# wwood/CoverM

Hardware: NVIDIA H100
Metric: reads/sec `coverm contig` (mean+trimmed_mean+covered_fraction) (higher is better)
Workload: dtype i32

## Files before the change

### coverm_b200/csrc/cmb_bgzf.cu

```cuda
#include <algorithm>
#include <atomic>
#include <chrono>
#include <climits>
#include <cstdio>
#include <cstdlib>
#include <cstring>
#include <thread>

#include <zlib.h>

#include "cmb_context.cuh"
#include "cmb_bgzf.cuh"

namespace {
#include "cmb_common.cuh"
#include "cmb_decode.cuh"
#include "cmb_decode_g8.cuh"
#include "cmb_decode_t1.cuh"
#include "cmb_pairs.cuh"
#include "cmb_filter.cuh"
}

namespace {
constexpr size_t DEC_COPY_CHUNK = 8u << 20;
constexpr size_t DEC_WINDOW_BYTES = 32u << 20;
size_t dec_window_bytes() {
  static const size_t v = [] {
    const char* e = getenv("CMB_DECODE_WINDOW_KB");
    const long kb = e ? atol(e) : 0;
    return kb > 0 ? (size_t)kb << 10 : DEC_WINDOW_BYTES;
  }();
  return v;
}
constexpr size_t DEC_SLACK = 1024;
constexpr const char* NM_PANIC = "Mapping record encountered that does not have an 'NM' auxiliary tag in the SAM/BAM format. This is "
                                 "required to work out some coverage statistics";
constexpr size_t DEC_FRONT = 256;

constexpr uint32_t T1_MIN_BLOCKS = 28000;
int inflate_kind(uint32_t n_blocks) {
  static const int forced = [] {
    const char* e = getenv("CMB_INFLATE");
    if (e && !strcmp(e, "t1")) return 0;
    if (e && !strcmp(e, "g8")) return 1;
    if (e && !strcmp(e, "w1")) return 2;
    return -1;
  }();
  if (forced >= 0) return forced;
  return n_blocks >= T1_MIN_BLOCKS ? 0 : 1;
}
bool inflate_serial_requested() {
  static const bool v = [] {
    if (const char* e = getenv("CMB_INFLATE_SERIAL")) return e[0] == '1';
    for (const char* name : {"CUDA_INJECTION64_PATH", "NV_NSIGHT_INJECTION_PORT_BASE", "NV_COMPUTE_PROFILER_PERFWORKS_DIR", "NV_SANITIZER_INJECTION_PORT_BASE"})
      if (const char* e = getenv(name))
        if (e[0]) return true;
    return false;
  }();
  return v;
}
int launch_crc32(cmb_ctx* c, const InflateArgs& a, cudaStream_t st) {
  const uint32_t nb = a.b1 - a.b0;
  kd_crc32<<<std::min<uint32_t>((nb + 7) / 8, (uint32_t)c->sm_count * 8), 256, 0, st>>>(a);
  CU_TRY(c, cudaGetLastError());
  return CMB_OK;
}
int launch_inflate(cmb_ctx* c, const InflateArgs& a, cudaStream_t st, bool* crc_pending = nullptr) {
  const uint32_t nb = a.b1 - a.b0;
  const int k = a.block_list ? 2 : inflate_kind(nb);
  if (k == 0) {
    CU_TRY(c, cudaFuncSetAttribute(kd_inflate_t1, cudaFuncAttributeMaxDynamicSharedMemorySize, (int)T1_SMEM_BYTES));
    const uint32_t max_grid = (uint32_t)c->sm_count * 5, warps = max_grid * (T1_THREADS / 32);
    const uint32_t lanes = std::min<uint32_t>(32, std::max<uint32_t>(1, (nb + warps - 1) / warps));
    const uint32_t per_cta = lanes * (T1_THREADS / 32);
    const uint32_t grid = std::min<uint32_t>((nb + per_cta - 1) / per_cta, max_grid);
    InflateArgs at = a;
    at.lane_limit = lanes;
    kd_inflate_t1<<<grid, T1_THREADS, T1_SMEM_BYTES, st>>>(at);
    CU_TRY(c, cudaGetLastError());
    if (crc_pending) *crc_pending = true;
    else if (int rc = launch_crc32(c, a, st)) return rc;
  } else if (k == 1) {
    CU_TRY(c, cudaFuncSetAttribute(kd_inflate_g8, cudaFuncAttributeMaxDynamicSharedMemorySize, (int)G8_SMEM_BYTES));
    const uint32_t per_cta = G8_WARPS * G8_STREAMS;
    const uint32_t grid = std::min<uint32_t>((nb + per_cta - 1) / per_cta, (uint32_t)c->sm_count * 2);
    kd_inflate_g8<<<grid, G8_WARPS * 32, G8_SMEM_BYTES, st>>>(a);
  } else {
    CU_TRY(c, cudaFuncSetAttribute(kd_inflate, cudaFuncAttributeMaxDynamicSharedMemorySize, (int)INF_SMEM_BYTES));
    const uint32_t grid = std::min<uint32_t>((nb + INF_WARPS - 1) / INF_WARPS, (uint32_t)c->sm_count * 2);
    kd_inflate<<<grid, INF_WARPS * 32, INF_SMEM_BYTES, st>>>(a);
  }
  CU_TRY(c, cudaGetLastError());
  return CMB_OK;
}

bool host_inflate_block(const cmb_bgzf_input* in, uint32_t b, std::vector<uint8_t>& buf) {
  const uint32_t isz = in->block_isize[b];
  if (buf.size() < (size_t)isz + 64) buf.resize((size_t)isz + 64);
  z_stream zs;
  memset(&zs, 0, sizeof zs);
  if (inflateInit2(&zs, -15) != Z_OK) return false;
  zs.next_in = const_cast<Bytef*>(in->data + in->block_coffset[b]);
  zs.avail_in = in->block_clen[b];
  zs.next_out = buf.data();
  zs.avail_out = isz;
  const bool ok = inflate(&zs, Z_FINISH) == Z_STREAM_END && zs.avail_out == 0;
  inflateEnd(&zs);
  uint32_t want_crc;
  memcpy(&want_crc, in->data + in->block_coffset[b] + in->block_clen[b], 4);
  return ok && (uint32_t)crc32(0, buf.data(), isz) == want_crc;
}

InflateArgs inflate_args(const BgzfCall& j, uint32_t b0, uint32_t b1) {
  const auto& d = j.d;
  InflateArgs a{};
  a.comp = j.comp_base; a.coff = d.d_coff; a.clen = d.d_clen; a.isize = d.d_isize; a.uoff = d.d_ustart; a.scratch = d.d_t1_scratch;
  a.b0 = b0; a.b1 = b1; a.out = j.infl_base; a.status = d.d_status; a.ticket = d.d_tickets; a.fail_count = d.d_cnt + 0;
  return a;
}

}

std::optional<uint64_t> cmb::decode_mem_limit() {
  const char* lim = getenv("CMB_DECODE_MEM_LIMIT_MB");
  if (!lim) return std::nullopt;
  return (uint64_t)(std::max(0.0, strtod(lim, nullptr)) * 1048576.0);
}

uint64_t cmb::decode_bytes(const cmb_ctx* c) {
  const auto& d = c->dec;
  return d.d_comp.bytes() + d.d_inflated.bytes() + d.d_tuple_slab.bytes() + d.d_rec_off.bytes() + c->sh.d_scan.bytes();
}

void cmb::release_decode(cmb_ctx* c) {
  cudaGetLastError();
  auto& d = c->dec;
  d.d_comp.release();
  d.d_inflated.release();
  d.d_tuple_slab.release();
  d.d_rec_off.release();
  c->sh.d_scan.release();
}

uint64_t cmb::device_room(uint64_t held) {
  if (const uint64_t lim = decode_mem_limit().value_or(0)) return lim;
  size_t free_b = 0, total_b = 0;
  cudaMemGetInfo(&free_b, &total_b);
  cudaGetLastError();
  return free_b + held;
}


int BgzfCall::run() {
  int rc = prepare();
  if (!rc && !nothing_to_decode && !(rc = copy_inflate()) && !(rc = declined()) && !(rc = chain())) rc = extract();
  return rc;
}

int BgzfCall::prepare() {
  ustart.assign((size_t)nb + 1, 0);
  for (uint32_t b = 0; b < nb; ++b) {
    if (in->block_coffset[b] + in->block_clen[b] + 8 > in->size) return fail(c, CMB_E_ARG, "cmb_submit_bgzf: block %u lies outside the data", b);
    ustart[b + 1] = ustart[b] + in->block_isize[b];
  }
  const uint64_t stream_total = ustart[nb];
  if (in->records_at > stream_total) return fail(c, CMB_E_ARG, "cmb_submit_bgzf: records_at beyond the end of the stream");
  if (in->records_at == stream_total) return CMB_OK;
  first_block = (uint32_t)(std::upper_bound(ustart.begin(), ustart.end(), in->records_at) - ustart.begin()) - 1;
  walk_end = data_end = nb;
  if (in->ranged) {
    if (in->walk_begin_block != first_block || in->walk_end_block > nb || in->walk_end_block < in->walk_begin_block)
      return fail(c, CMB_E_ARG, "cmb_submit_bgzf: inconsistent block range");
    walk_end = in->walk_end_block;
    if (walk_end == first_block) return CMB_OK;
    data_end = walk_end;
    uint64_t tail = 0;
    while (data_end < nb && tail < tail_bytes) tail += in->block_isize[data_end++];
  }
  nothing_to_decode = false;
  byte_lo = in->block_coffset[first_block];
  byte_hi = data_end == nb ? in->size : in->block_coffset[data_end - 1] + in->block_clen[data_end - 1] + 8;
  u_lo = ustart[first_block];
  total = ustart[data_end];
  if (const auto lim = decode_mem_limit())
    if (((byte_hi - byte_lo) + (total - u_lo)) >> 20 > *lim >> 20) return CMB_E_NOMEM;
  int rc;
  const size_t comp_need = (size_t)(byte_hi - byte_lo) + DEC_FRONT + DEC_SLACK, infl_need = (size_t)(total - u_lo) + DEC_SLACK;
  if ((rc = d.d_comp.ensure(c, comp_need, with_slack(comp_need))) || (rc = d.d_inflated.ensure(c, infl_need, with_slack(infl_need))))
    return rc;
  comp_base = reinterpret_cast<uint8_t*>(reinterpret_cast<uintptr_t>(d.d_comp.p) + DEC_FRONT - byte_lo);
  infl_base = reinterpret_cast<uint8_t*>(reinterpret_cast<uintptr_t>(d.d_inflated.p) - u_lo);
  const size_t blocks_need = (size_t)nb + 1, blocks_want = (size_t)nb + nb / 8 + 64;
  for (auto* b : {&d.d_coff, &d.d_ustart, &d.d_guess, &d.d_exit, &d.d_rec_base, &d.d_cig_base})
    if ((rc = b->ensure(c, blocks_need, blocks_want))) return rc;
  for (auto* b : {&d.d_clen, &d.d_isize, &d.d_status, &d.d_nrec, &d.d_ncig, &d.d_dirty})
    if ((rc = b->ensure(c, blocks_need, blocks_want))) return rc;
  if ((rc = d.d_t1_scratch.ensure(c, blocks_need * T1_LENS_BYTES, blocks_want * T1_LENS_BYTES))) return rc;
  if ((rc = d.d_cnt.ensure(c, 20))) return rc;
  if (!d.have_events) {
    for (auto& e : d.ev) CU_TRY(c, cudaEventCreate(&e));
    d.have_events = true;
  }
  {
    uint32_t b = first_block;
    uint64_t byte0 = byte_lo;
    while (b < data_end) {
      uint32_t e = b;
      uint64_t byte1 = byte0;
      while (e < data_end && (e == b || in->block_coffset[e] + in->block_clen[e] + 8 - byte0 <= dec_window_bytes())) {
        byte1 = in->block_coffset[e] + in->block_clen[e] + 8;
        ++e;
      }
      if (e == data_end) byte1 = byte_hi;
      windows.push_back({b, e, byte0, byte1});
      b = e;
      byte0 = byte1;
    }
  }
  const size_t n_windows = windows.size();
  if ((rc = d.d_tickets.ensure(c, n_windows + 8, n_windows * 3 + 64))) return rc;
  if ((rc = d.d_block_window.ensure(c, nb, with_slack(nb)))) return rc;
  if (!d.h_ones) {
    if ((rc = d.h_ones.ensure(c, 16))) return rc;
    for (int k = 0; k < 16; ++k) d.h_ones.p[k] = 1;
  }
  cudaPointerAttributes attr{};
  src_pinned = cudaPointerGetAttributes(&attr, in->data) == cudaSuccess && attr.type == cudaMemoryTypeHost;
  cudaGetLastError();
  const uint32_t T = std::min<uint32_t>(std::min<uint32_t>(in->copy_threads ? in->copy_threads : 4, 16), (uint32_t)n_windows);
  n_copy_threads = T;
  while (d.streams.size() < T) {
    cudaStream_t st;
    CU_TRY(c, cudaStreamCreateWithFlags(&st, cudaStreamNonBlocking));
    d.streams.push_back(st);
    cudaEvent_t e;
    CU_TRY(c, cudaEventCreateWithFlags(&e, cudaEventDisableTiming));
    d.done_events.push_back(e);
    for (int k = 0; k < 2; ++k) {
      CU_TRY(c, cudaEventCreateWithFlags(&e, cudaEventDisableTiming));
      d.slot_events.push_back(e);
      PinnedBuf<uint8_t> slot;
      if ((rc = slot.ensure(c, DEC_COPY_CHUNK))) return rc;
      d.pinned.push_back(std::move(slot));
    }
  }
  return CMB_OK;
}

int BgzfCall::copy_inflate() {
  NvtxRange nvtx("bgzf: H2D copy + inflate");
  const uint32_t T = n_copy_threads;
  std::vector<uint32_t> block_window(nb, 0);
  for (size_t w = 0; w < windows.size(); ++w)
    for (uint32_t b = windows[w].b0; b < windows[w].b1; ++b) block_window[b] = (uint32_t)w;
  CU_TRY(c, cudaEventRecord(d.ev[0], c->stream));
  CU_TRY(c, cudaMemcpyAsync(d.d_coff, in->block_coffset, 8ull * nb, cudaMemcpyHostToDevice, c->stream));
  CU_TRY(c, cudaMemcpyAsync(d.d_clen, in->block_clen, 4ull * nb, cudaMemcpyHostToDevice, c->stream));
  CU_TRY(c, cudaMemcpyAsync(d.d_isize, in->block_isize, 4ull * nb, cudaMemcpyHostToDevice, c->stream));
  CU_TRY(c, cudaMemcpyAsync(d.d_ustart, ustart.data(), 8ull * (nb + 1), cudaMemcpyHostToDevice, c->stream));
  CU_TRY(c, cudaMemsetAsync(d.d_cnt, 0, 64, c->stream));
  CU_TRY(c, cudaMemsetAsync(d.d_status, 0, 4ull * nb, c->stream));
  CU_TRY(c, cudaMemcpyAsync(d.d_block_window, block_window.data(), 4ull * nb, cudaMemcpyHostToDevice, c->stream));
  CU_TRY(c, cudaMemsetAsync(d.d_tickets, 0, 4 * (windows.size() + 1), c->stream));
  CU_TRY(c, cudaMemsetAsync(infl_base + total, 0, DEC_SLACK, c->stream));
  CU_TRY(c, cudaMemsetAsync(comp_base + byte_hi, 0, DEC_SLACK, c->stream));
  CU_TRY(c, cudaMemsetAsync(d.d_comp, 0, DEC_FRONT, c->stream));
  CU_TRY(c, cudaEventRecord(d.ev[1], c->stream));
  for (uint32_t t = 0; t < T; ++t) CU_TRY(c, cudaStreamWaitEvent(d.streams[t], d.ev[1], 0));
  const bool serial = windows.size() <= 1 || inflate_serial_requested();
  bool crc_pending = false;
  InflateArgs persistent = inflate_args(*this, first_block, data_end);
  int rc;
  if (!serial) {
    persistent.block_window = d.d_block_window;
    persistent.ready = d.d_tickets + 1;
    if ((rc = launch_inflate(c, persistent, c->stream, &crc_pending))) return rc;
  }
  std::atomic<size_t> next_window{0};
  std::atomic<int> first_err{0};
  auto worker = [&](uint32_t t) {
    cudaSetDevice(c->device);
    cudaStream_t st = d.streams[t];
    int slot = 0;
    bool used[2] = {false, false};
    auto check = [&](cudaError_t e) {
      if (e != cudaSuccess) {
        int z = 0;
        first_err.compare_exchange_strong(z, (int)e);
      }
      return e == cudaSuccess;
    };
    for (;;) {
      const size_t w = next_window.fetch_add(1);
      if (w >= windows.size() || first_err.load()) break;
      const Window& win = windows[w];
      if (src_pinned) {
        if (!check(cudaMemcpyAsync(comp_base + win.byte0, in->data + win.byte0, win.byte1 - win.byte0, cudaMemcpyHostToDevice, st))) break;
      } else {
        for (uint64_t o = win.byte0; o < win.byte1; o += DEC_COPY_CHUNK) {
          const size_t n = (size_t)std::min<uint64_t>(DEC_COPY_CHUNK, win.byte1 - o);
          const size_t si = (size_t)t * 2 + slot;
          if (used[slot] && !check(cudaEventSynchronize(d.slot_events[si]))) return;
          memcpy(d.pinned[si], in->data + o, n);
          if (!check(cudaMemcpyAsync(comp_base + o, d.pinned[si], n, cudaMemcpyHostToDevice, st))) return;
          if (!check(cudaEventRecord(d.slot_events[si], st))) return;
          used[slot] = true;
          slot ^= 1;
        }
      }
      if (!check(cudaMemcpyAsync(d.d_tickets + 1 + w, d.h_ones, 4, cudaMemcpyHostToDevice, st))) break;
    }
    check(cudaEventRecord(d.done_events[t], st));
  };
  const auto copy_t0 = std::chrono::steady_clock::now();
  {
    std::vector<std::thread> threads;
    for (uint32_t t = 1; t < T; ++t) threads.emplace_back(worker, t);
    worker(0);
    for (auto& th : threads) th.join();
  }
  const double copy_wall_ms = std::chrono::duration<double, std::milli>(std::chrono::steady_clock::now() - copy_t0).count();
  out->ms_copy_enqueue_wall = (float)copy_wall_ms;
  if (crc_pending && (rc = launch_crc32(c, persistent, c->stream))) return rc;
  if (serial && !first_err.load()) {
    for (uint32_t t = 0; t < T; ++t) CU_TRY(c, cudaStreamWaitEvent(c->stream, d.done_events[t], 0));
    if ((rc = launch_inflate(c, inflate_args(*this, first_block, data_end), c->stream))) return rc;
  }
  if (first_err.load()) {
    cudaMemsetAsync(d.d_tickets + 1, 1, 4 * windows.size(), d.streams[0]);
    cudaStreamSynchronize(d.streams[0]);
    cudaStreamSynchronize(c->stream);
  }
  out->n_launches = 1;
  out->h2d_bytes = (byte_hi - byte_lo) + 24ull * nb + 8;
  if (first_err.load()) return fail(c, CMB_E_CUDA, "cmb_submit_bgzf: copy/inflate stage failed: %s", cudaGetErrorString((cudaError_t)first_err.load()));
  for (uint32_t t = 0; t < T; ++t) CU_TRY(c, cudaStreamWaitEvent(c->stream, d.done_events[t], 0));
  if (getenv("CMB_PIPELINE_STATS")) {
    const auto h0 = std::chrono::steady_clock::now();
    for (uint32_t t = 0; t < T; ++t) cudaEventSynchronize(d.done_events[t]);
    const double wait_ms = std::chrono::duration<double, std::milli>(std::chrono::steady_clock::now() - h0).count();
    fprintf(stderr, "#decode_h2d\twindows=%zu\tbytes=%llu\tcopy_streams_done_after_ms=%.1f (host clock from the end of the enqueue; enqueue took %.1f ms)\n",
            windows.size(), (unsigned long long)(byte_hi - byte_lo), wait_ms, copy_wall_ms);
  }
  CU_TRY(c, cudaEventRecord(d.ev[2], c->stream));
  if (getenv("CMB_DECODE_PROFILE")) {
    CU_TRY(c, cudaStreamSynchronize(c->stream));
    cudaEvent_t p0, p1;
    cudaEventCreate(&p0);
    cudaEventCreate(&p1);
    CU_TRY(c, cudaMemsetAsync(d.d_tickets, 0, 4, c->stream));
    InflateArgs a = inflate_args(*this, first_block, data_end);
    a.fail_count = d.d_cnt + 8;
    cudaEventRecord(p0, c->stream);
    if ((rc = launch_inflate(c, a, c->stream))) return rc;
    cudaEventRecord(p1, c->stream);
    CU_TRY(c, cudaStreamSynchronize(c->stream));
    float ms = 0;
    cudaEventElapsedTime(&ms, p0, p1);
    fprintf(stderr, "#decode_profile\tinflate_only_ms=%.3f\tblocks=%u\tcompressed=%llu\tinflated=%llu\tinflated_GBps=%.2f\tcopy_threads=%u\tsrc_pinned=%d\tcopy_enqueue_wall_ms=%.2f\n", ms, data_end - first_block,
            (unsigned long long)(byte_hi - byte_lo), (unsigned long long)(total - u_lo), (total - u_lo) / ms * 1e-6, T, (int)src_pinned, copy_wall_ms);
    cudaEventDestroy(p0);
    cudaEventDestroy(p1);
  }
  return CMB_OK;
}

int BgzfCall::declined() {
  NvtxRange nvtx("bgzf: declined blocks (second pass, host zlib)");
  uint32_t h_cnt[16];
  CU_TRY(c, cudaMemcpyAsync(h_cnt, d.d_cnt, 64, cudaMemcpyDeviceToHost, c->stream));
  CU_TRY(c, cudaStreamSynchronize(c->stream));
  std::vector<uint8_t> tmp;
  if (h_cnt[0] || getenv("CMB_DECODE_RETRY_TEST")) {
    std::vector<uint32_t> status(nb);
    CU_TRY(c, cudaMemcpy(status.data(), d.d_status, 4ull * nb, cudaMemcpyDeviceToHost));
    if (getenv("CMB_DECODE_RETRY_TEST"))
      for (uint32_t b = first_block; b < data_end; b += 7) status[b] = 29;
    if (getenv("CMB_DECODE_VERIFY") || getenv("CMB_PIPELINE_STATS")) {
      uint32_t hist[32] = {0};
      for (uint32_t b = 0; b < nb; ++b) hist[std::min<uint32_t>(status[b], 31)]++;
      fprintf(stderr, "#decode_status");
      for (int k = 0; k < 32; ++k)
        if (hist[k]) fprintf(stderr, "\t%d:%u", k, hist[k]);
      fprintf(stderr, "\n");
    }
    std::vector<uint32_t> again;
    for (uint32_t b = first_block; b < data_end; ++b)
      if (status[b] != INF_OK) again.push_back(b);
    out->n_blocks_second_pass = (uint32_t)again.size();
    if (!again.empty()) {
      uint32_t* d_list = d.d_dirty;
      CU_TRY(c, cudaMemcpyAsync(d_list, again.data(), 4ull * again.size(), cudaMemcpyHostToDevice, c->stream));
      CU_TRY(c, cudaMemsetAsync(d.d_tickets, 0, 4, c->stream));
      CU_TRY(c, cudaMemsetAsync(d.d_cnt, 0, 4, c->stream));
      InflateArgs a = inflate_args(*this, 0, (uint32_t)again.size());
      a.block_list = d_list;
      if (int rc = launch_inflate(c, a, c->stream)) return rc;
      out->n_launches += 1;
      std::vector<uint32_t> st2(nb);
      CU_TRY(c, cudaMemcpyAsync(st2.data(), d.d_status, 4ull * nb, cudaMemcpyDeviceToHost, c->stream));
      CU_TRY(c, cudaStreamSynchronize(c->stream));
      for (uint32_t b : again) status[b] = st2[b];
    }
    for (uint32_t b = first_block; b < data_end; ++b) {
      if (status[b] == INF_OK) continue;
      if (!host_inflate_block(in, b, tmp)) return fail(c, CMB_E_DECLINED, "cmb_submit_bgzf: BGZF block %u does not inflate", b);
      CU_TRY(c, cudaMemcpy(infl_base + ustart[b], tmp.data(), in->block_isize[b], cudaMemcpyHostToDevice));
      out->n_blocks_host += 1;
    }
  }
  if (getenv("CMB_DECODE_VERIFY")) {
    std::vector<uint8_t> dev(total - u_lo);
    CU_TRY(c, cudaMemcpy(dev.data(), d.d_inflated, total - u_lo, cudaMemcpyDeviceToHost));
    uint32_t bad = 0;
// ... 285 lines not shown
      if ((rc = pair_cut(j, filter_out, carry, j.walk_end >= walk_end, who, host_route, &largest, &cut, next))) return rc;
      ss.ms_mates += std::chrono::duration<float, std::milli>(std::chrono::steady_clock::now() - t0).count();
    }
    if ((rc = work(j, r, cut))) return rc;
    carry = largest;
    ss.pair_cut_records += n - cut;
    side = (double)other() / (double)std::max<uint64_t>(1, (j.byte_hi - j.byte_lo) + (j.total - j.u_lo));
    return CMB_OK;
  };
  auto nomem = [&](const SliceBlocks&, uint32_t, uint32_t, uint64_t) {
    return fail(c, CMB_E_DECLINED, "%s: not enough device memory for device-side decode", who);
  };
  const int rc = decode_in_slices(c, in, out, ss, budget, step, nomem);
  release_decode(c);
  if (rc) return rc;
  if (getenv("CMB_PIPELINE_STATS"))
    fprintf(stderr, "#%s_slices\tslices=%u\tmax_slice_bytes=%llu\thalvings=%u\tpair_cut_records=%llu\n", stats, ss.n_slices,
            (unsigned long long)ss.max_slice, ss.halvings, (unsigned long long)ss.pair_cut_records);
  return CMB_OK;
}

int decode_sliced(cmb_ctx* c, const cmb_bgzf_input* in, cmb_bgzf_result* out) {
  auto& d = c->dec;
  *out = cmb_bgzf_result{};
  const bool pair = c->mode.filter_pairs;
  auto work = [&](BgzfCall& j, cmb_bgzf_result& r, uint32_t cut) -> int {
    const uint32_t n = (uint32_t)j.n_rec;
    uint32_t iv_sub = (uint32_t)j.n_cig;
    cmb_read_batch tb;
    carve_batch(d.d_tuple_slab, n, (uint32_t)j.n_cig, &tb);
    if (cut < n) {
      CU_TRY(c, cudaMemcpyAsync(&iv_sub, tb.iv_begin + cut, 4, cudaMemcpyDeviceToHost, c->stream));
      CU_TRY(c, cudaMemsetAsync(d.d_cnt + 16, 0, 16, c->stream));
      kd_count_held<<<(n - cut + 255) / 256, 256, 0, c->stream>>>(tb.tid, tb.flag, cut, n, j.in->own_tid_begin, j.in->own_tid_end, j.in->own_unplaced,
                                                                 (unsigned long long*)(d.d_cnt + 16), (unsigned long long*)(d.d_cnt + 18));
      CU_TRY(c, cudaGetLastError());
      uint64_t held[2] = {0, 0};
      CU_TRY(c, cudaMemcpyAsync(held, d.d_cnt + 16, 16, cudaMemcpyDeviceToHost, c->stream));
      CU_TRY(c, cudaStreamSynchronize(c->stream));
      r.n_primary -= held[0];
      r.n_records -= held[1];
      r.n_intervals = iv_sub;
      r.n_launches += 1;
    }
    if (!k1_active(c)) return CMB_OK;
    uint32_t excl = 0;
    if (int rc = j.excl_n(&excl)) return rc;
    const int rc = launch_k1(c, tb, cut, iv_sub, excl, pair ? d.d_pair_mate.p : nullptr);
    return rc == CMB_E_NOMEM ? SLICE_HALVE : rc;
  };
  SliceStats ss;
  const int rc = stream_in_slices(
      c, in, out, ss, "cmb_submit_bgzf", "mates are matched on the host", "decode", pair, true, !c->gene_mode, [&] { return decode_bytes(c); },
      [&] { return d.d_tuple_slab.bytes() + d.d_rec_off.bytes() + (pair ? pair_bytes(c) : 0); }, work);
  if (rc == CMB_E_DECLINED)
    if (int e = reset_sample(c)) return e;
  if (rc) return rc;
  out->ms_copy_inflate = ss.ms_inflate;
  out->ms_chain = ss.ms_chain;
  out->ms_extract = ss.ms_extract;
  return CMB_OK;
}

int bgzf_entry(cmb_ctx* c, const cmb_bgzf_input* in, cmb_bgzf_result* out, bool decode_only) {
  if (c) {
    c->dec.last_valid = false;
    c->dec.filter_planned = false;
  }
  const auto t_call0 = std::chrono::steady_clock::now();
  const int rc = whole_or_slices(c, submit_bgzf_impl(c, in, out, decode_only), [&] {
    return decode_only ? fail(c, CMB_E_DECLINED, "cmb_submit_bgzf: not enough device memory for device-side decode") : decode_sliced(c, in, out);
  });
  if (out) out->ms_host_wall = (float)std::chrono::duration<double, std::milli>(std::chrono::steady_clock::now() - t_call0).count();
  return rc;
}

int filter_kernels(cmb_ctx* c, bool pair_path, int inverse, uint32_t n, uint64_t* total, uint64_t* n_emit) {
  auto& d = c->dec;
  int rc;
  if ((rc = d.d_filter_anchor.ensure(c, (size_t)n + 1, with_slack(n))) || (rc = d.d_filter_role.ensure(c, (size_t)n + 1, with_slack(n))))
    return rc;
  cmb_read_batch tb;
  carve_batch(d.d_tuple_slab, d.last_n_rec, d.last_n_cig, &tb);
  FilterArgs a{};
  a.data = d.last_infl_base; a.rec_off = d.d_rec_off; a.n = n; a.flag = tb.flag; a.mapq = tb.mapq; a.nm_state = tb.nm_state; a.nm = tb.nm;
  a.l_seq = tb.l_seq; a.aligned = tb.aligned; a.del = tb.del; a.mate = pair_path ? d.last_mate : nullptr; a.p = c->params;
  a.filter_single = c->mode.filter_single_reads; a.pair_path = pair_path; a.filter_out = inverse ? 0 : 1;
  a.anchor_bytes = d.d_filter_anchor; a.role = d.d_filter_role; a.error_flags = d.d_cnt + 12; a.n_emit = (unsigned long long*)(d.d_cnt + 14);
  CU_TRY(c, cudaMemsetAsync(d.d_cnt + 12, 0, 16, c->stream));
  kf_decide<<<(n + 255) / 256, 256, 0, c->stream>>>(a);
  kf_scan<<<1, 1024, 0, c->stream>>>(d.d_filter_anchor, n);
  CU_TRY(c, cudaGetLastError());
  uint32_t h[4];
  CU_TRY(c, cudaMemcpyAsync(h, d.d_cnt + 12, 16, cudaMemcpyDeviceToHost, c->stream));
  CU_TRY(c, cudaMemcpyAsync(total, d.d_filter_anchor + n, 8, cudaMemcpyDeviceToHost, c->stream));
  CU_TRY(c, cudaStreamSynchronize(c->stream));
  if (h[0] & ERR_NM) return fail(c, CMB_E_NM, "%s", NM_PANIC);
  memcpy(n_emit, h + 2, 8);
  if (!*total) return CMB_OK;
  if ((rc = d.d_filter_out.ensure(c, *total, (size_t)*total + (size_t)*total / 8 + 4096))) return rc;
  a.out = d.d_filter_out;
  kf_gather<<<(n + 7) / 8, 256, 0, c->stream>>>(a);
  CU_TRY(c, cudaGetLastError());
  return CMB_OK;
}
}

// ... 175 lines not shown
```

### coverm_b200/csrc/cmb_context.cuh

```cuda
#pragma once
#include <cuda.h>
#include <cuda_runtime.h>

#include <condition_variable>
#include <cstddef>
#include <cstdint>
#include <memory>
#include <mutex>
#include <string>
#include <utility>
#include <vector>

#include <nccl.h>
#include <nvtx3/nvToolsExt.h>

#include "../../include/coverm_b200.h"

namespace cmb __attribute__((visibility("hidden"))) {

struct NvtxRange {
  explicit NvtxRange(const char* name) { nvtxRangePushA(name); }
  ~NvtxRange() { nvtxRangePop(); }
  NvtxRange(const NvtxRange&) = delete;
  NvtxRange& operator=(const NvtxRange&) = delete;
// ... 89 lines not shown
  uint32_t next_batch = 0;
  uint32_t n_contigs = 0, tid_begin = 0, tid_end = 0, n_local = 0;
  uint64_t arena_elems = 0;
  uint32_t n_chunks = 0;
  struct Reference {
    Buf<int32_t> d_arena;
    Buf<uint32_t> d_span_bits;
    Buf<uint32_t> d_word_count, d_word_off, d_word_block_sum;
    Buf<uint32_t> d_off_span, d_len, d_chunk_first;
    Buf<int32_t> d_tail_sum, d_carry_in;
    Buf<int2> d_block_agg;
    Buf<cmb_contig_stats> d_rows;
    Buf<uint32_t> d_bins;
    Buf<uint64_t> d_bin_base, d_bin_block_sum;
    Buf<uint32_t> d_bin_hi;
    Buf<cmb_hist_pair> d_pairs;
    Buf<uint32_t> d_gene_first, d_gene_start, d_gene_end, d_gene_maxlen, d_contig_len32;
    Buf<uint8_t> d_contig_seen;
    Buf<uint32_t> d_gene_bound;
  } ref;
  Buf<uint32_t> d_counters;
  Buf<ulonglong2> d_events;
  Buf<uint16_t> d_buckets;
  uint32_t kept_range[2] = {0, 0};
  ncclComm_t comm = nullptr;
  int comm_rank = 0, comm_size = 1;
  std::shared_ptr<LocalBarrier> local_barrier;
  Buf<uint8_t> d_xchg;
  Buf<cmb_hist_pair> d_pairs_all;
  Buf<int2> d_block_minmax;
  Buf<int2> d_block_xrange;
  bool have_xrange = false;
  uint32_t block_minmax_used = 0;
  bool gene_mode = false;
  uint32_t n_ref_contigs = 0;
  uint32_t gene_tid_begin = 0, gene_tid_end = 0;
  CUtensorMap tmap{};
  bool arena_dirty = true;
  bool pool_dirty = false;
  bool clean_as_you_go = true;
  cmb_params params{};
  cmb_filter_mode mode{};
  bool have_params = false, in_sample = false, ended = false;
  cudaEvent_t ev[8]{};
  cmb_sample_timing timing{};
  std::vector<std::pair<cudaEvent_t, cudaEvent_t>> k1_events;
  uint32_t k1_events_used = 0;
  uint64_t n_records = 0, n_intervals = 0;
  struct Decode {
    Buf<uint8_t> d_comp, d_inflated;
    Buf<uint64_t> d_coff, d_ustart, d_guess, d_exit, d_rec_base, d_cig_base;
    Buf<uint32_t> d_clen, d_isize, d_status, d_nrec, d_ncig, d_dirty;
    Buf<uint8_t> d_t1_scratch;
    Buf<uint32_t> d_tickets;
    Buf<uint32_t> d_block_window;
    PinnedBuf<uint32_t> h_ones;
    Buf<uint32_t> d_cnt;
    Buf<uint64_t> d_rec_off;
    Buf<uint8_t> d_tuple_slab;
    uint32_t last_n_rec = 0, last_n_cig = 0;
    bool last_valid = false;
    Buf<uint64_t> d_pair_key;
    Buf<int32_t> d_pair_mate;
    Buf<uint32_t> d_pair_next;
    Buf<unsigned long long> d_pair_tag;
    Buf<uint32_t> d_pair_head;
    Buf<uint2> d_pair_order;
    const int32_t* last_mate = nullptr;
    bool last_mate_inverse = false;
    uint32_t last_excl_n = 0xffffffffu;
    const uint8_t* last_infl_base = nullptr;
    Buf<unsigned long long> d_filter_anchor;
    Buf<uint8_t> d_filter_role;
    Buf<uint8_t> d_filter_out;
    uint64_t filter_bytes = 0;
    bool filter_planned = false;
    PinnedBuf<uint8_t> filter_stage[2];
    std::vector<PinnedBuf<uint8_t>> pinned;
    std::vector<cudaStream_t> streams;
    std::vector<cudaEvent_t> slot_events, done_events;
    cudaEvent_t ev[6]{};
    bool have_events = false;
  } dec;
  struct Shards {
    struct Store {
      Buf<int32_t> tid, pos, iv_start, iv_len;
      Buf<uint32_t> nm, l_seq, aligned, del, ins, iv_begin;
      Buf<uint16_t> flag;
      Buf<uint8_t> mapq, nm_state, info;
      Buf<unsigned long long> names;
      Buf<int32_t> as_val;
      Buf<uint8_t> as_state;
      ShardStore view{};
      uint64_t n_prim = 0, n_iv = 0;
      uint64_t bytes() const {
        return tid.bytes() + pos.bytes() + iv_start.bytes() + iv_len.bytes() + nm.bytes() + l_seq.bytes() + aligned.bytes() + del.bytes() +
               ins.bytes() + iv_begin.bytes() + flag.bytes() + mapq.bytes() + nm_state.bytes() + info.bytes() + names.bytes() +
               as_val.bytes() + as_state.bytes();
      }
    };
    std::vector<Store> store;
    std::vector<int32_t> tid_offsets;
    uint32_t n_shards = 0, added = 0;
    bool active = false;
    uint32_t first = 0, last = 0;
    bool group = false;
// ... 130 lines not shown
```

### coverm_b200/csrc/cmb_decode_t1.cuh

```cuda
#pragma once

constexpr uint32_t T1_THREADS = 96;

struct T1Stream {
  uint8_t perm_lit_lo[288];
  uint32_t perm_lit_hi[9];
  int16_t base_lit[16];
  int16_t base_dst[16];
  uint16_t tmp[16];
  uint8_t perm_dst[32];
};
static_assert(sizeof(T1Stream) == 452, "T1Stream layout");
constexpr uint32_t T1_SMEM_BYTES = T1_THREADS * sizeof(T1Stream);
constexpr uint32_t T1_LENS_BYTES = 160;

struct T1Reader {
  const uint32_t* wp;
  uint32_t w0, w1;
  uint64_t buf;
  uint32_t cnt;
  __device__ __forceinline__ void init(const uint8_t* p) {
    const uintptr_t a = (uintptr_t)p;
    wp = reinterpret_cast<const uint32_t*>(a & ~(uintptr_t)3);
    const uint32_t skip = (uint32_t)(a & 3) * 8;
    buf = (uint64_t)(__ldcg(wp++) >> skip);
    cnt = 32 - skip;
    w0 = __ldcg(wp++);
    w1 = __ldcg(wp++);
    refill();
  }
  __device__ __forceinline__ void refill() {
    const bool take = cnt <= 32;
    if (take) {
      buf |= (uint64_t)w0 << cnt;
      cnt += 32;
      w0 = w1;
    }
#ifdef __CUDA_ARCH__
    asm volatile(
        "{\n"
        ".reg .pred p;\n"
        "setp.ne.u32 p, %2, 0;\n"
        "@p ld.global.cg.u32 %0, [%1];\n"
        "}\n"
        : "+r"(w1)
        : "l"(wp), "r"((uint32_t)take)
        : "memory");
#else
    if (take) w1 = __ldcg(wp);
#endif
    if (take) ++wp;
  }
  __device__ __forceinline__ void consume(uint32_t n) {
    buf >>= n;
    cnt -= n;
  }
  __device__ __forceinline__ uint32_t bits(uint32_t n) const { return (uint32_t)buf & ((1u << n) - 1); }
  __device__ __forceinline__ uint32_t peek15() const { return __brev((uint32_t)buf) >> 17; }
  __device__ __forceinline__ const uint8_t* byte_pos_ceil() const { return reinterpret_cast<const uint8_t*>(wp - 2) - (cnt >> 3); }
};

__device__ __forceinline__ uint32_t t1_code_len(uint32_t p, const uint32_t (&lim)[15]) {
  uint32_t L = 1;
#pragma unroll
  for (int k = 0; k < 15; ++k) L += p >= lim[k] ? 1u : 0u;
  return L;
}

template <class LenOf, class Put>
__device__ __forceinline__ bool t1_build(LenOf len_of, uint32_t n, Put put, int16_t* base, uint16_t* tmp, uint32_t (&lim)[15]) {
#pragma unroll
  for (int L = 0; L < 16; ++L) tmp[L] = 0;
  for (uint32_t s = 0; s < n; ++s) tmp[len_of(s)] += 1;
  uint32_t code = 0, off = 0, prev = 0;
  int left = 1;
  bool ok = true;
#pragma unroll
  for (int L = 1; L <= 15; ++L) {
    const uint32_t c = tmp[L];
    code = (code + prev) << 1;
    left = left * 2 - (int)c;
    if (left < 0) {
      ok = false;
      left = 0;
    }
    lim[L - 1] = (code + c) << (15 - L);
    base[L] = (int16_t)((int)off - (int)code);
    tmp[L] = (uint16_t)off;
    off += c;
    prev = c;
  }
  for (uint32_t s = 0; s < n; ++s) {
    const uint32_t l = len_of(s);
    if (l) put((uint32_t)tmp[l]++, s);
  }
  return ok;
}

constexpr unsigned long long T1_WAIT_NS = 2000000000ull;
#ifndef T1_HOST_TEST
__device__ __forceinline__ unsigned long long t1_now_ns() {
  unsigned long long t;
  asm volatile("mov.u64 %0, %%globaltimer;" : "=l"(t));
  return t;
}
__device__ __forceinline__ void t1_lane_busy(volatile uint32_t* w, int d) { atomicAdd(const_cast<uint32_t*>(w), (uint32_t)d); }
#else
static inline unsigned long long t1_now_ns() { return 0; }
static inline void t1_lane_busy(volatile uint32_t* w, int d) { *w += (uint32_t)d; }
static inline void __syncwarp() {}
#endif
__global__ void __launch_bounds__(T1_THREADS, 5) kd_inflate_t1(const InflateArgs a) {
  extern __shared__ __align__(16) uint8_t t1_smem[];
  T1Stream& S = reinterpret_cast<T1Stream*>(t1_smem)[threadIdx.x];
  uint32_t lit_lim[15], dst_lim[15];
#pragma unroll
  for (int k = 0; k < 15; ++k) lit_lim[k] = dst_lim[k] = 0;
  T1Reader br;
  br.wp = nullptr;
  br.w0 = br.w1 = 0;
  br.buf = 0;
  br.cnt = 0;

  uint32_t pm_len = 0;
  uint8_t* pm_dp = nullptr;
  uint8_t pm[8] = {0, 0, 0, 0, 0, 0, 0, 0};
  auto flush_pending = [&]() {
    if (pm_len) {
#pragma unroll
      for (uint32_t k = 0; k < 8; ++k)
        if (k < pm_len) pm_dp[k] = pm[k];
      pm_len = 0;
    }
  };
  enum : uint32_t { IDLE, WAIT, HDR, SYM, FIN };
  uint32_t state = IDLE;
  uint32_t b = 0, n_out = 0, op = 0, bfinal = 0, spins = 0, skip = 0;
  unsigned long long wait_t0 = 0;
  __shared__ uint32_t t1_busy[T1_THREADS / 32];
  volatile uint32_t* const my_busy = t1_busy + (threadIdx.x >> 5);
  if ((threadIdx.x & 31) == 0) *my_busy = 0;
  __syncwarp();
  bool counted = false;
  const uint8_t* in_end = nullptr;
  uint8_t* out = nullptr;

  if (a.lane_limit && (threadIdx.x & 31) >= a.lane_limit) return;
  for (;;) {
    if (state == IDLE) {
      const uint32_t tk = atomicAdd(a.ticket, 1u);
      if (tk >= a.b1 - a.b0) return;
      b = a.block_list ? a.block_list[tk] : a.b0 + tk;
      spins = 0;
      skip = 0;
      wait_t0 = 0;
      state = WAIT;
    }
    if (state == WAIT && skip) {
      --skip;
    } else if (state == WAIT) {
      bool arrived = true;
      if (a.ready) arrived = *(const volatile uint32_t*)(a.ready + a.block_window[b]) != 0;
      if (arrived) {
        if (a.ready) __threadfence_system();
        n_out = a.isize[b];
        const uint8_t* in = a.comp + a.coff[b];
        in_end = in + a.clen[b];
        out = a.out + a.uoff[b];
        op = 0;
        if (n_out == 0) {
          a.status[b] = 0;
          state = IDLE;
        } else {
          br.init(in);
          state = HDR;
          t1_lane_busy(my_busy, 1);
          counted = true;
        }
      } else {
        const unsigned long long now = t1_now_ns();
        if (wait_t0 == 0) wait_t0 = now;
        if (now - wait_t0 > T1_WAIT_NS) {
          a.status[b] = 31u;
          atomicAdd(a.fail_count, 1u);
          state = IDLE;
        } else if (*my_busy == 0) {
          __nanosleep(256u << (spins < 4u ? spins : 4u));
          ++spins;
        } else {
          skip = 512;
        }
      }
    }
    uint32_t st = 0;
    if (state == HDR) {
      if (br.byte_pos_ceil() > in_end) st = 1;
      br.refill();
      bfinal = br.bits(1);
      const uint32_t btype = ((uint32_t)br.buf >> 1) & 3;
      br.consume(3);
      if (st == 0 && btype == 3) st = 4;
      if (st == 0 && btype == 0) {
        br.consume(br.cnt & 7);
        br.refill();
        const uint32_t len = (uint32_t)br.buf & 0xffff, nlen = ((uint32_t)br.buf >> 16) & 0xffff;
        br.consume(32);
        const uint8_t* src = br.byte_pos_ceil();
        if ((len ^ nlen) != 0xffff) st = 2;
        else if (src + len > in_end || op + len > n_out) st = 3;
        else {
          for (uint32_t i = 0; i < len; ++i) out[op + i] = __ldcg(src + i);
          op += len;
          br.init(src + len);
        }
        if (st == 0 && bfinal) state = FIN;
      } else if (st == 0) {
        uint8_t* const l4 = a.scratch + (size_t)b * T1_LENS_BYTES;
        uint32_t hlit = 288, hdist = 32;
        if (btype == 1) {
          for (uint32_t i = 0; i < 160; ++i) {
            const uint32_t s0 = 2 * i, s1 = 2 * i + 1;
            auto fl = [](uint32_t s) -> uint32_t { return s < 144 ? 8u : s < 256 ? 9u : s < 280 ? 7u : s < 288 ? 8u : 5u; };
            l4[i] = (uint8_t)(fl(s0) | (fl(s1) << 4));
          }
        } else {
          br.refill();
          hlit = br.bits(5) + 257;
          hdist = (((uint32_t)br.buf >> 5) & 31) + 1;
          const uint32_t hclen = (((uint32_t)br.buf >> 10) & 15) + 4;
          br.consume(14);
          if (hlit > 286 || hdist > 30) st = 5;
          if (st == 0) {
            for (uint32_t i = 0; i < 10; ++i) l4[150 + i] = 0;
            for (uint32_t i = 0; i < hclen; ++i) {
              br.refill();
              const uint32_t sym = c_clen_order[i], v = br.bits(3);
              br.consume(3);
              l4[150 + (sym >> 1)] |= (uint8_t)(v << ((sym & 1) * 4));
            }
            uint8_t* pd = S.perm_dst;
            const bool okc = t1_build([l4](uint32_t s) -> uint32_t { return (l4[150 + (s >> 1)] >> ((s & 1) * 4)) & 15u; }, 19u,
                                      [pd](uint32_t i, uint32_t s) { pd[i] = (uint8_t)s; }, S.base_dst, S.tmp, dst_lim);
            if (!okc) st = 6;
          }
          if (st == 0) {
            const uint32_t total = hlit + hdist;
            uint32_t n = 0, prev = 0;
            auto put = [&](uint32_t i, uint32_t v) {
              const uint32_t sh = (i & 1) * 4;
              l4[i >> 1] = (uint8_t)((l4[i >> 1] & ~(15u << sh)) | (v << sh));
            };
            while (n < total && st == 0) {
              br.refill();
              const uint32_t p = br.peek15();
              const uint32_t L = t1_code_len(p, dst_lim);
              if (L > 7) {
                st = 7;
                break;
              }
              const uint32_t sym = S.perm_dst[(int)S.base_dst[L] + (int)(p >> (15 - L))];
              br.consume(L);
              if (sym < 16) {
                put(n, sym);
                prev = sym;
                ++n;
// ... 16 lines not shown
                }
                if (n + rep > total) {
                  st = 9;
                  break;
                }
                for (uint32_t i = 0; i < rep; ++i) put(n + i, val);
                prev = val;
                n += rep;
              }
            }
            if (st == 0 && ((l4[128] & 15u) == 0)) st = 10;
          }
        }
        if (st == 0) {
          const uint32_t hl = hlit;
          uint8_t* pd = S.perm_dst;
          uint8_t* plo = S.perm_lit_lo;
          uint32_t* phi = S.perm_lit_hi;
#pragma unroll
          for (int k = 0; k < 9; ++k) phi[k] = 0;
          const bool okd = t1_build([l4, hl](uint32_t s) -> uint32_t { const uint32_t i = hl + s; return (l4[i >> 1] >> ((i & 1) * 4)) & 15u; }, hdist,
                                    [pd](uint32_t i, uint32_t s) { pd[i] = (uint8_t)s; }, S.base_dst, S.tmp, dst_lim);
          const bool okl = t1_build([l4](uint32_t s) -> uint32_t { return (l4[s >> 1] >> ((s & 1) * 4)) & 15u; }, hlit,
                                    [plo, phi](uint32_t i, uint32_t s) {
                                      plo[i] = (uint8_t)s;
                                      if (s & 256u) phi[i >> 5] |= 1u << (i & 31);
                                    },
                                    S.base_lit, S.tmp, lit_lim);
          if (!okd) st = 11;
          else if (!okl) st = 12;
          else state = SYM;
        }
      }
    }
    if (state == SYM && st == 0) {
      if (br.byte_pos_ceil() > in_end + 8) st = 21;
#pragma unroll 1
      for (int pass = 0; pass < 16 && st == 0; ++pass) {
        br.refill();
        uint32_t p = br.peek15();
        uint32_t L = t1_code_len(p, lit_lim);
        if (L > 15) {
          st = 13;
          break;
        }
        const uint32_t li = (uint32_t)((int)S.base_lit[L] + (int)(p >> (15 - L)));
        const uint32_t sym = (uint32_t)S.perm_lit_lo[li] | (((S.perm_lit_hi[li >> 5] >> (li & 31)) & 1u) << 8);
        br.consume(L);
        if (sym < 256) {
          if (op >= n_out) {
            st = 14;
            break;
          }
          out[op++] = (uint8_t)sym;
          continue;
        }
        if (sym == 256) {
          state = bfinal ? FIN : HDR;
          break;
        }
        const uint32_t c = sym - 257;
        if (c > 28) {
          st = 15;
          break;
        }
        uint32_t len, xl = 0;
        if (c < 8) len = 3 + c;
        else if (c == 28) len = 258;
        else {
          xl = (c >> 2) - 1;
          len = 3 + ((4 + (c & 3)) << xl);
        }
        len += br.bits(xl);
        br.consume(xl);
        br.refill();
        p = br.peek15();
        L = t1_code_len(p, dst_lim);
        if (L > 15) {
          st = 16;
          break;
        }
        const uint32_t d = S.perm_dst[(int)S.base_dst[L] + (int)(p >> (15 - L))];
        br.consume(L);
        if (d > 29) {
          st = 17;
          break;
        }
        uint32_t dist, xd = 0;
        if (d < 4) dist = 1 + d;
        else {
          xd = (d >> 1) - 1;
          dist = 1 + ((2 + (d & 1)) << xd);
        }
        dist += br.bits(xd);
        br.consume(xd);
        if (dist > op || op + len > n_out) {
          st = 18;
          break;
        }
        uint8_t* dp = out + op;
        const uint8_t* sp = dp - dist;
        flush_pending();
        if (len <= 8 && dist >= len) {
#pragma unroll
          for (uint32_t k = 0; k < 8; ++k)
            if (k < len) pm[k] = sp[k];
          pm_len = len;
          pm_dp = dp;
        } else if (dist >= len) {
          for (uint32_t i = 0; i < len; i += 8) {
            uint8_t t8[8];
#pragma unroll
            for (uint32_t k = 0; k < 8; ++k)
              if (i + k < len) t8[k] = sp[i + k];
#pragma unroll
            for (uint32_t k = 0; k < 8; ++k)
              if (i + k < len) dp[i + k] = t8[k];
          }
        } else {
          for (uint32_t i = 0; i < len; ++i) dp[i] = sp[i];
        }
        op += len;
      }
      flush_pending();
    }
    if (state == FIN && st == 0) {
      if (op != n_out) st = 19;
      else if (br.byte_pos_ceil() > in_end) st = 20;
      if (st == 0) {
        a.status[b] = 0;
        state = IDLE;
      }
    }
    if (st != 0) {
      a.status[b] = st;
      atomicAdd(a.fail_count, 1u);
      state = IDLE;
    }
    if (state == IDLE && counted) {
      t1_lane_busy(my_busy, -1);
      counted = false;
    }
  }
}

#ifndef T1_HOST_TEST
__global__ void __launch_bounds__(256) kd_crc32(const InflateArgs a) {
  __shared__ uint32_t crcT[1024];
  {
    uint32_t c = threadIdx.x;
    for (int k = 0; k < 8; ++k) c = (c & 1) ? (c >> 1) ^ CRC_POLY : c >> 1;
    crcT[threadIdx.x] = c;
  }
  __syncthreads();
  {
    uint32_t c = crcT[threadIdx.x];
    for (int k = 1; k < 4; ++k) {
      c = crcT[c & 0xff] ^ (c >> 8);
      crcT[k * 256 + threadIdx.x] = c;
    }
  }
  __syncthreads();
  const uint32_t lane = threadIdx.x & 31;
  const uint32_t warps = gridDim.x * 8;
  for (uint32_t i = blockIdx.x * 8 + (threadIdx.x >> 5); i < a.b1 - a.b0; i += warps) {
    const uint32_t b = a.block_list ? a.block_list[i] : a.b0 + i;
    const uint32_t n = a.isize[b];
    if (n == 0 || a.status[b] != 0) continue;
    const uint8_t* f = a.comp + a.coff[b] + a.clen[b];
    const uint32_t want = (uint32_t)__ldcg(f) | ((uint32_t)__ldcg(f + 1) << 8) | ((uint32_t)__ldcg(f + 2) << 16) | ((uint32_t)__ldcg(f + 3) << 24);
    const uint32_t got = warp_crc32(a.out + a.uoff[b], n, crcT, lane);
    if (got != want && lane == 0) {
      a.status[b] = 30u;
      atomicAdd(a.fail_count, 1u);
    }
  }
}
#endif
```

Measured before the change: 5.452 billion.

## Defer T1 inflate match copies to warp-parallel resolve pass fused with CRC

The T1 inflate kernel no longer copies LZ77 back-references inline. It writes literals through an 8-byte accumulator with aligned stores and records each match (literal run, length, distance) in a per-block list in a new device buffer. The CRC kernel becomes a resolve kernel: it prefix-scans match offsets across a warp, replays matches in dependency-safe waves, then checks the CRC. This takes dependent byte-by-byte copies off the serial Huffman decode loop, at the cost of extra device memory, an extra pass over the output, and a new failure status when the match list overflows.

```diff
diff --git a/coverm_b200/csrc/cmb_bgzf.cu b/coverm_b200/csrc/cmb_bgzf.cu
--- a/coverm_b200/csrc/cmb_bgzf.cu
+++ b/coverm_b200/csrc/cmb_bgzf.cu
@@ -59,13 +59,13 @@
   }();
   return v;
 }
-int launch_crc32(cmb_ctx* c, const InflateArgs& a, cudaStream_t st) {
+int launch_t1_resolve(cmb_ctx* c, const InflateArgs& a, cudaStream_t st) {
   const uint32_t nb = a.b1 - a.b0;
-  kd_crc32<<<std::min<uint32_t>((nb + 7) / 8, (uint32_t)c->sm_count * 8), 256, 0, st>>>(a);
+  kd_t1_resolve<<<std::min<uint32_t>((nb + 7) / 8, (uint32_t)c->sm_count * 8), 256, 0, st>>>(a, c->dec.d_t1_matches);
   CU_TRY(c, cudaGetLastError());
   return CMB_OK;
 }
-int launch_inflate(cmb_ctx* c, const InflateArgs& a, cudaStream_t st, bool* crc_pending = nullptr) {
+int launch_inflate(cmb_ctx* c, const InflateArgs& a, cudaStream_t st, bool* resolve_pending = nullptr) {
   const uint32_t nb = a.b1 - a.b0;
   const int k = a.block_list ? 2 : inflate_kind(nb);
   if (k == 0) {
@@ -76,10 +76,10 @@
     const uint32_t grid = std::min<uint32_t>((nb + per_cta - 1) / per_cta, max_grid);
     InflateArgs at = a;
     at.lane_limit = lanes;
-    kd_inflate_t1<<<grid, T1_THREADS, T1_SMEM_BYTES, st>>>(at);
+    kd_inflate_t1<<<grid, T1_THREADS, T1_SMEM_BYTES, st>>>(at, c->dec.d_t1_matches);
     CU_TRY(c, cudaGetLastError());
-    if (crc_pending) *crc_pending = true;
-    else if (int rc = launch_crc32(c, a, st)) return rc;
+    if (resolve_pending) *resolve_pending = true;
+    else if (int rc = launch_t1_resolve(c, a, st)) return rc;
   } else if (k == 1) {
     CU_TRY(c, cudaFuncSetAttribute(kd_inflate_g8, cudaFuncAttributeMaxDynamicSharedMemorySize, (int)G8_SMEM_BYTES));
     const uint32_t per_cta = G8_WARPS * G8_STREAMS;
@@ -129,7 +129,7 @@
 
 uint64_t cmb::decode_bytes(const cmb_ctx* c) {
   const auto& d = c->dec;
-  return d.d_comp.bytes() + d.d_inflated.bytes() + d.d_tuple_slab.bytes() + d.d_rec_off.bytes() + c->sh.d_scan.bytes();
+  return d.d_comp.bytes() + d.d_inflated.bytes() + d.d_t1_matches.bytes() + d.d_tuple_slab.bytes() + d.d_rec_off.bytes() + c->sh.d_scan.bytes();
 }
 
 void cmb::release_decode(cmb_ctx* c) {
@@ -137,6 +137,7 @@
   auto& d = c->dec;
   d.d_comp.release();
   d.d_inflated.release();
+  d.d_t1_matches.release();
   d.d_tuple_slab.release();
   d.d_rec_off.release();
   c->sh.d_scan.release();
@@ -196,6 +197,10 @@
   for (auto* b : {&d.d_clen, &d.d_isize, &d.d_status, &d.d_nrec, &d.d_ncig, &d.d_dirty})
     if ((rc = b->ensure(c, blocks_need, blocks_want))) return rc;
   if ((rc = d.d_t1_scratch.ensure(c, blocks_need * T1_LENS_BYTES, blocks_want * T1_LENS_BYTES))) return rc;
+  if (inflate_kind(data_end - first_block) == 0) {
+    const size_t words = t1_list_words(total - u_lo, data_end - first_block);
+    if ((rc = d.d_t1_matches.ensure(c, words, with_slack(words)))) return rc;
+  }
   if ((rc = d.d_cnt.ensure(c, 20))) return rc;
   if (!d.have_events) {
     for (auto& e : d.ev) CU_TRY(c, cudaEventCreate(&e));
@@ -268,13 +273,13 @@
   CU_TRY(c, cudaEventRecord(d.ev[1], c->stream));
   for (uint32_t t = 0; t < T; ++t) CU_TRY(c, cudaStreamWaitEvent(d.streams[t], d.ev[1], 0));
   const bool serial = windows.size() <= 1 || inflate_serial_requested();
-  bool crc_pending = false;
+  bool resolve_pending = false;
   InflateArgs persistent = inflate_args(*this, first_block, data_end);
   int rc;
   if (!serial) {
     persistent.block_window = d.d_block_window;
     persistent.ready = d.d_tickets + 1;
-    if ((rc = launch_inflate(c, persistent, c->stream, &crc_pending))) return rc;
+    if ((rc = launch_inflate(c, persistent, c->stream, &resolve_pending))) return rc;
   }
   std::atomic<size_t> next_window{0};
   std::atomic<int> first_err{0};
@@ -321,7 +326,7 @@
   }
   const double copy_wall_ms = std::chrono::duration<double, std::milli>(std::chrono::steady_clock::now() - copy_t0).count();
   out->ms_copy_enqueue_wall = (float)copy_wall_ms;
-  if (crc_pending && (rc = launch_crc32(c, persistent, c->stream))) return rc;
+  if (resolve_pending && (rc = launch_t1_resolve(c, persistent, c->stream))) return rc;
   if (serial && !first_err.load()) {
     for (uint32_t t = 0; t < T; ++t) CU_TRY(c, cudaStreamWaitEvent(c->stream, d.done_events[t], 0));
     if ((rc = launch_inflate(c, inflate_args(*this, first_block, data_end), c->stream))) return rc;
@@ -351,15 +356,22 @@
     CU_TRY(c, cudaMemsetAsync(d.d_tickets, 0, 4, c->stream));
     InflateArgs a = inflate_args(*this, first_block, data_end);
     a.fail_count = d.d_cnt + 8;
+    cudaEvent_t pm;
+    cudaEventCreate(&pm);
+    bool resolve = false;
     cudaEventRecord(p0, c->stream);
-    if ((rc = launch_inflate(c, a, c->stream))) return rc;
+    if ((rc = launch_inflate(c, a, c->stream, &resolve))) return rc;
+    cudaEventRecord(pm, c->stream);
+    if (resolve && (rc = launch_t1_resolve(c, a, c->stream))) return rc;
     cudaEventRecord(p1, c->stream);
     CU_TRY(c, cudaStreamSynchronize(c->stream));
-    float ms = 0;
+    float ms = 0, ms_first = 0;
     cudaEventElapsedTime(&ms, p0, p1);
-    fprintf(stderr, "#decode_profile\tinflate_only_ms=%.3f\tblocks=%u\tcompressed=%llu\tinflated=%llu\tinflated_GBps=%.2f\tcopy_threads=%u\tsrc_pinned=%d\tcopy_enqueue_wall_ms=%.2f\n", ms, data_end - first_block,
+    cudaEventElapsedTime(&ms_first, p0, pm);
+    fprintf(stderr, "#decode_profile\tinflate_only_ms=%.3f\tfirst_kernel_ms=%.3f\tblocks=%u\tcompressed=%llu\tinflated=%llu\tinflated_GBps=%.2f\tcopy_threads=%u\tsrc_pinned=%d\tcopy_enqueue_wall_ms=%.2f\n", ms, ms_first, data_end - first_block,
             (unsigned long long)(byte_hi - byte_lo), (unsigned long long)(total - u_lo), (total - u_lo) / ms * 1e-6, T, (int)src_pinned, copy_wall_ms);
     cudaEventDestroy(p0);
+    cudaEventDestroy(pm);
     cudaEventDestroy(p1);
   }
   return CMB_OK;
@@ -751,7 +763,7 @@
   SliceStats ss;
   const int rc = stream_in_slices(
       c, in, out, ss, "cmb_submit_bgzf", "mates are matched on the host", "decode", pair, true, !c->gene_mode, [&] { return decode_bytes(c); },
-      [&] { return d.d_tuple_slab.bytes() + d.d_rec_off.bytes() + (pair ? pair_bytes(c) : 0); }, work);
+      [&] { return d.d_t1_matches.bytes() + d.d_tuple_slab.bytes() + d.d_rec_off.bytes() + (pair ? pair_bytes(c) : 0); }, work);
   if (rc == CMB_E_DECLINED)
     if (int e = reset_sample(c)) return e;
   if (rc) return rc;
diff --git a/coverm_b200/csrc/cmb_context.cuh b/coverm_b200/csrc/cmb_context.cuh
--- a/coverm_b200/csrc/cmb_context.cuh
+++ b/coverm_b200/csrc/cmb_context.cuh
@@ -165,6 +165,7 @@
     Buf<uint64_t> d_coff, d_ustart, d_guess, d_exit, d_rec_base, d_cig_base;
     Buf<uint32_t> d_clen, d_isize, d_status, d_nrec, d_ncig, d_dirty;
     Buf<uint8_t> d_t1_scratch;
+    Buf<uint32_t> d_t1_matches;
     Buf<uint32_t> d_tickets;
     Buf<uint32_t> d_block_window;
     PinnedBuf<uint32_t> h_ones;
diff --git a/coverm_b200/csrc/cmb_decode_t1.cuh b/coverm_b200/csrc/cmb_decode_t1.cuh
--- a/coverm_b200/csrc/cmb_decode_t1.cuh
+++ b/coverm_b200/csrc/cmb_decode_t1.cuh
@@ -13,6 +13,38 @@
 static_assert(sizeof(T1Stream) == 452, "T1Stream layout");
 constexpr uint32_t T1_SMEM_BYTES = T1_THREADS * sizeof(T1Stream);
 constexpr uint32_t T1_LENS_BYTES = 160;
+
+#ifndef T1_MATCH_DIV
+#define T1_MATCH_DIV 3
+#endif
+constexpr uint32_t T1_ST_MATCH_LIST = 22;
+__device__ __forceinline__ uint32_t t1_list_cap(uint32_t isize) { return isize / T1_MATCH_DIV + 1; }
+__device__ __forceinline__ size_t t1_list_at(const InflateArgs& a, uint32_t b) {
+  return (size_t)((a.uoff[b] - a.uoff[a.b0]) / T1_MATCH_DIV) + 2ull * (b - a.b0);
+}
+inline size_t t1_list_words(uint64_t inflated, uint32_t n_blocks) { return (size_t)(inflated / T1_MATCH_DIV) + 2ull * n_blocks + 2; }
+
+struct T1Match {
+  uint32_t lit, len, dist;
+};
+__device__ __forceinline__ T1Match t1_match(uint32_t e) { return {e >> 24, (e >> 15) & 511u, (e & 0x7fffu) + 1}; }
+__device__ __forceinline__ uint32_t t1_src_end(uint32_t op, const T1Match& m) { return op - m.dist + (m.len < m.dist ? m.len : m.dist); }
+__device__ __forceinline__ void t1_copy_match(uint8_t* d, uint32_t dist, uint32_t len) {
+  const uint8_t* s = d - dist;
+  uint32_t r = 0;
+  for (uint32_t i = 0; i < len; i += 16) {
+    uint8_t t[16];
+#pragma unroll
+    for (uint32_t k = 0; k < 16; ++k)
+      if (i + k < len) {
+        t[k] = s[r];
+        r = r + 1 == dist ? 0 : r + 1;
+      }
+#pragma unroll
+    for (uint32_t k = 0; k < 16; ++k)
+      if (i + k < len) d[i + k] = t[k];
+  }
+}
 
 struct T1Reader {
   const uint32_t* wp;
@@ -110,7 +142,7 @@
 static inline void t1_lane_busy(volatile uint32_t* w, int d) { *w += (uint32_t)d; }
 static inline void __syncwarp() {}
 #endif
-__global__ void __launch_bounds__(T1_THREADS, 5) kd_inflate_t1(const InflateArgs a) {
+__global__ void __launch_bounds__(T1_THREADS, 5) kd_inflate_t1(const InflateArgs a, uint32_t* matches) {
   extern __shared__ __align__(16) uint8_t t1_smem[];
   T1Stream& S = reinterpret_cast<T1Stream*>(t1_smem)[threadIdx.x];
   uint32_t lit_lim[15], dst_lim[15];
@@ -122,17 +154,6 @@
   br.buf = 0;
   br.cnt = 0;
 
-  uint32_t pm_len = 0;
-  uint8_t* pm_dp = nullptr;
-  uint8_t pm[8] = {0, 0, 0, 0, 0, 0, 0, 0};
-  auto flush_pending = [&]() {
-    if (pm_len) {
-#pragma unroll
-      for (uint32_t k = 0; k < 8; ++k)
-        if (k < pm_len) pm_dp[k] = pm[k];
-      pm_len = 0;
-    }
-  };
   enum : uint32_t { IDLE, WAIT, HDR, SYM, FIN };
   uint32_t state = IDLE;
   uint32_t b = 0, n_out = 0, op = 0, bfinal = 0, spins = 0, skip = 0;
@@ -144,6 +165,27 @@
   bool counted = false;
   const uint8_t* in_end = nullptr;
   uint8_t* out = nullptr;
+  uint64_t acc = 0;
+  uint32_t o7 = 0;
+  auto flush = [&](uint32_t at) {
+    const uintptr_t lo = (uintptr_t)out, hi = lo + n_out, w = (lo + at) & ~(uintptr_t)7;
+    if (w >= lo && w + 8 <= hi) {
+      *reinterpret_cast<uint64_t*>(w) = acc;
+    } else {
+#pragma unroll
+      for (uint32_t k = 0; k < 8; ++k)
+        if (w + k >= lo && w + k < hi) *reinterpret_cast<uint8_t*>(w + k) = (uint8_t)(acc >> (8 * k));
+    }
+    acc = 0;
+  };
+  auto put = [&](uint32_t v) {
+    const uint32_t ph = (o7 + op) & 7;
+    acc |= (uint64_t)v << (8 * ph);
+    if (ph == 7) flush(op);
+    ++op;
+  };
+  uint32_t* ml = nullptr;
+  uint32_t n_m = 0, m_cap = 0, m_end = 0;
 
   if (a.lane_limit && (threadIdx.x & 31) >= a.lane_limit) return;
   for (;;) {
@@ -168,6 +210,11 @@
         in_end = in + a.clen[b];
         out = a.out + a.uoff[b];
         op = 0;
+        acc = 0;
+        o7 = (uint32_t)(uintptr_t)out & 7;
+        ml = matches + t1_list_at(a, b);
+        n_m = m_end = 0;
+        m_cap = t1_list_cap(n_out);
         if (n_out == 0) {
           a.status[b] = 0;
           state = IDLE;
@@ -209,8 +256,7 @@
         if ((len ^ nlen) != 0xffff) st = 2;
         else if (src + len > in_end || op + len > n_out) st = 3;
         else {
-          for (uint32_t i = 0; i < len; ++i) out[op + i] = __ldcg(src + i);
-          op += len;
+          for (uint32_t i = 0; i < len; ++i) put(__ldcg(src + i));
           br.init(src + len);
         }
         if (st == 0 && bfinal) state = FIN;
@@ -333,7 +379,7 @@
             st = 14;
             break;
           }
-          out[op++] = (uint8_t)sym;
+          put(sym);
           continue;
         }
         if (sym == 256) {
@@ -379,36 +425,28 @@
           st = 18;
           break;
         }
-        uint8_t* dp = out + op;
-        const uint8_t* sp = dp - dist;
-        flush_pending();
-        if (len <= 8 && dist >= len) {
-#pragma unroll
-          for (uint32_t k = 0; k < 8; ++k)
-            if (k < len) pm[k] = sp[k];
-          pm_len = len;
-          pm_dp = dp;
-        } else if (dist >= len) {
-          for (uint32_t i = 0; i < len; i += 8) {
-            uint8_t t8[8];
-#pragma unroll
-            for (uint32_t k = 0; k < 8; ++k)
-              if (i + k < len) t8[k] = sp[i + k];
-#pragma unroll
-            for (uint32_t k = 0; k < 8; ++k)
-              if (i + k < len) dp[i + k] = t8[k];
-          }
-        } else {
-          for (uint32_t i = 0; i < len; ++i) dp[i] = sp[i];
-        }
+        uint32_t lit = op - m_end;
+        while (lit > 255 && n_m < m_cap) {
+          ml[1 + n_m++] = 255u << 24;
+          lit -= 255;
+        }
+        if (n_m >= m_cap) {
+          st = T1_ST_MATCH_LIST;
+          break;
+        }
+        ml[1 + n_m++] = lit << 24 | len << 15 | (dist - 1);
+        const uint32_t ph = (o7 + op) & 7;
+        if (ph != 0 && ph + len >= 8) flush(op);
         op += len;
-      }
-      flush_pending();
+        m_end = op;
+      }
     }
     if (state == FIN && st == 0) {
       if (op != n_out) st = 19;
       else if (br.byte_pos_ceil() > in_end) st = 20;
       if (st == 0) {
+        if ((o7 + op) & 7) flush(op);
+        ml[0] = n_m;
         a.status[b] = 0;
         state = IDLE;
       }
@@ -426,35 +464,65 @@
 }
 
 #ifndef T1_HOST_TEST
-__global__ void __launch_bounds__(256) kd_crc32(const InflateArgs a) {
+__global__ void __launch_bounds__(256) kd_t1_resolve(const InflateArgs a, const uint32_t* matches) {
   __shared__ uint32_t crcT[1024];
-  {
-    uint32_t c = threadIdx.x;
-    for (int k = 0; k < 8; ++k) c = (c & 1) ? (c >> 1) ^ CRC_POLY : c >> 1;
-    crcT[threadIdx.x] = c;
-  }
-  __syncthreads();
-  {
-    uint32_t c = crcT[threadIdx.x];
-    for (int k = 1; k < 4; ++k) {
-      c = crcT[c & 0xff] ^ (c >> 8);
-      crcT[k * 256 + threadIdx.x] = c;
-    }
-  }
+  crc32_fill_tables(crcT, threadIdx.x);
   __syncthreads();
   const uint32_t lane = threadIdx.x & 31;
   const uint32_t warps = gridDim.x * 8;
   for (uint32_t i = blockIdx.x * 8 + (threadIdx.x >> 5); i < a.b1 - a.b0; i += warps) {
-    const uint32_t b = a.block_list ? a.block_list[i] : a.b0 + i;
+    const uint32_t b = a.b0 + i;
     const uint32_t n = a.isize[b];
     if (n == 0 || a.status[b] != 0) continue;
+    uint8_t* const out = a.out + a.uoff[b];
+    const uint32_t* const ml = matches + t1_list_at(a, b);
+    const uint32_t nm = ml[0];
+    uint32_t base = 0;
+    for (uint32_t k0 = 0; k0 < nm; k0 += 32) {
+      const T1Match m = t1_match(k0 + lane < nm ? ml[1 + k0 + lane] : 0u);
+      uint32_t end = m.lit + m.len;
+#pragma unroll
+      for (uint32_t d = 1; d < 32; d <<= 1) {
+        const uint32_t o = __shfl_up_sync(FULL, end, d);
+        if (lane >= d) end += o;
+      }
+      end += base;
+      base = __shfl_sync(FULL, end, 31);
+      const uint32_t op = end - m.len;
+      uint32_t waiting = __ballot_sync(FULL, m.len != 0);
+      while (waiting) {
+        const uint32_t first = __shfl_sync(FULL, op, __ffs(waiting) - 1);
+        const bool go = ((waiting >> lane) & 1) && t1_src_end(op, m) <= first;
+        if (go) t1_copy_match(out + op, m.dist, m.len);
+        __syncwarp();
+        waiting &= ~__ballot_sync(FULL, go);
+      }
+    }
     const uint8_t* f = a.comp + a.coff[b] + a.clen[b];
     const uint32_t want = (uint32_t)__ldcg(f) | ((uint32_t)__ldcg(f + 1) << 8) | ((uint32_t)__ldcg(f + 2) << 16) | ((uint32_t)__ldcg(f + 3) << 24);
-    const uint32_t got = warp_crc32(a.out + a.uoff[b], n, crcT, lane);
+    const uint32_t got = warp_crc32(out, n, crcT, lane);
     if (got != want && lane == 0) {
       a.status[b] = 30u;
       atomicAdd(a.fail_count, 1u);
     }
   }
 }
+#else
+static inline void kd_inflate_t1(const InflateArgs& a) {
+  uint64_t span = 0;
+  for (uint32_t b = a.b0; b < a.b1; ++b) span = std::max<uint64_t>(span, a.uoff[b] + a.isize[b] - a.uoff[a.b0]);
+  std::vector<uint32_t> matches(t1_list_words(span, a.b1 - a.b0), 0xdeadbeefu);
+  kd_inflate_t1(a, matches.data());
+  for (uint32_t b = a.b0; b < a.b1; ++b) {
+    if (a.isize[b] == 0 || a.status[b] != 0) continue;
+    const uint32_t* ml = matches.data() + t1_list_at(a, b);
+    uint32_t op = 0;
+    for (uint32_t k = 0; k < ml[0]; ++k) {
+      const T1Match m = t1_match(ml[1 + k]);
+      op += m.lit;
+      t1_copy_match(a.out + a.uoff[b] + op, m.dist, m.len);
+      op += m.len;
+    }
+  }
+}
 #endif
```

Measured after the change: 5.453 billion (median of 6 runs). About the same (+0.0%).
